# olivesgatech/R3D

Hardware: AMD Instinct MI355X
Metric: training clips/sec (RGB+Depth fusion, DARai) at 1/2/4/8 GPUs; effective-rank match (higher is better)
Workload: dtype f32 (depth products: bf16x3 split on the bf16 matrix cores, fp32 accumulate)

## Files before the change

r3d_amd/csrc/decoder_chain.hip:

```cpp
#include "chain_bf3.h"
#include "mha_small.h"
#include "losses_dev.h"

namespace r3d {

constexpr int kDcBufA = 0;
constexpr int kDcBufB = kDcBufA + kFcRows * kFcP1;
constexpr int kDcBufF = kDcBufB + kFcRows * kFcP1;
constexpr int kDcWl = kDcBufF + kFcRows * kFcP4;
constexpr int kDcWlWave = 128 * kFbWP;
constexpr int kDcRed = kDcWl + 8 * kDcWlWave;
constexpr int kDcLdsFloats = kDcRed + 2 * 2 * 8 * kFcRows;
constexpr int kDcLdsBytes = kDcLdsFloats * 4;
static_assert(16 * kFcWP <= kDcWlWave && mha_small_lds_floats(16, 8) <= kDcWlWave && mha_small_bwd_lds_floats(16, 8) <= kDcWlWave,
              "wave region");
static_assert(kDcLdsBytes + (2 * 8 * (kTLHeads + 8) + 8 * 4 * 128 + 64) * 4 <= 160 * 1024, "LDS (dynamic + the tail's static arrays)");

typedef r3d_decoder_chain_args DcArgs;

__device__ __forceinline__ void dc_stage_rows(float* buf, const float* src, int row0, int tid) {
    const int r = tid >> 5, c4 = tid & 31;
    const f32x4 z = {0.f, 0.f, 0.f, 0.f};
    const f32x4 v = *reinterpret_cast<const f32x4*>(src + (size_t)(row0 + (r & 7)) * kFcH + 4 * c4);
    *reinterpret_cast<f32x4*>(buf + r * kFcP1 + 4 * c4) = r < 8 ? v : z;
// ... 427 lines not shown
            if (CHIP) relu |= (f > 0.f ? 1u : 0u) << (4 * t + i);
        }
    }
    if (CHIP) {
        keep.relu = relu;
#pragma unroll
        for (int t = 0; t < 4; ++t)
            keep.kbf[t] = kbf[t];
    }
    __syncthreads();
    R3D_CHAIN_MARK(D.timeline, b == 0, 5);
    acc0 = zero; acc1 = zero;
    bf3_chunk<4>(imgF, kD3P4, li, q, 0, b2, acc0, acc1);
    __builtin_amdgcn_sched_barrier(0);
    bf3_bload<4>(b2, D.pl_w2, 16, wave, 12, lane);
    __builtin_amdgcn_sched_barrier(0);
    bf3_chunk<4>(imgF, kD3P4, li, q, 4, b0, acc0, acc1);
    bf3_chunk<4>(imgF, kD3P4, li, q, 8, b1, acc0, acc1);
    bf3_chunk<4>(imgF, kD3P4, li, q, 12, b2, acc0, acc1);
    if (live) {
#pragma unroll
        for (int i = 0; i < 4; ++i) {
            const float v = ((acc0[i] + acc1[i]) + b_2) * md3.keep((uint8_t)(kb3 >> (8 * i)), D.drop_scale) + t2v[i];
            D.t3_pre[(size_t)(row0 + 4 * q + i) * H + c] = v;
            if (CHIP) scr0[kD3Xt + (4 * q + i) * H + c] = v;
        }
    }
}

struct Dc3TailIo {
    static constexpr bool kChip = true;
    float* scr0; unsigned short* imgA; const unsigned short* pl_w2_t; int tid_, wave, lane;
    Bf3B& w0; Bf3B& w1;
    __device__ __forceinline__ int tid() const { return tid_; }
    __device__ __forceinline__ float x(int row, int c) const { return scr0[kD3Xt + row * kFcH + c]; }
    __device__ __forceinline__ float ln(int which, int c) const { return scr0[kD3Par + which * kFcH + c]; }
    __device__ __forceinline__ float wh(int k, int c) const { return scr0[kD3ParWh + k * kFcH + c]; }
    __device__ __forceinline__ float bh(int k) const { return scr0[kD3ParBh + k]; }
    __device__ __forceinline__ void grads(int row, int c, float dx, float dx2) const {
        scr0[kD3Dxt + row * kFcH + c] = dx;
        asm volatile("" : "+v"(dx2));
        bf3_store1(imgA, kD3P1, row, c, dx2);
    }
    __device__ __forceinline__ void loads_requested() const {
        bf3_bload<4>(w0, pl_w2_t, 4, 4 * wave + 0, 0, lane);
        bf3_bload<4>(w1, pl_w2_t, 4, 4 * wave + 1, 0, lane);
    }
};

template <bool CHIP>
__device__ __forceinline__ void dc3_bwd(const DcArgs& D, const int b_, float* lds, const Dc3Keep& keep, Bf3B& b0, Bf3B& b1, Bf3B& b2) {
    int tid = threadIdx.x, b = b_;
    if (CHIP) { asm volatile("" : "+v"(tid)); asm volatile("" : "+s"(b)); }
    const int lane = tid & 63, wave = tid >> 6;
    const int li = lane & 15, q = lane >> 4;
    unsigned short* img = reinterpret_cast<unsigned short*>(lds);
    unsigned short* imgA = img + kD3ImgA;
    unsigned short* imgF = img + kD3ImgF;
    float* dct = reinterpret_cast<float*>(img + kD3ImgB);
    float* scr0 = reinterpret_cast<float*>(reinterpret_cast<unsigned char*>(lds) + kD3ScrBytes);
    float* scr = scr0 + wave * kD3ScrWave;
    float* redA = reinterpret_cast<float*>(reinterpret_cast<unsigned char*>(lds) + kD3RedBytes);
    constexpr int H = kFcH;
    const int row0 = b * 8;
    const int c = wave * 16 + li;
    const bool live = q < 2;
    const f32x4 zero = {0.f, 0.f, 0.f, 0.f};
// ... 102 lines not shown
            const float o = r2v[i] * (g[i] - s1v[i] - xh[i] * s2v[i]);
            const size_t e = (size_t)(row0 + 4 * q + i) * H + c;
            const float ok = o * md2.keep(kb2[i], D.drop_scale);
            if (live) { D.d_t2pre[e] = o; D.d_cap[e] = ok; }
            bf3_store1(imgA, kD3P1, 4 * q + i, c, live ? ok : 0.f);
        }
    }
    __syncthreads();
    R3D_CHAIN_MARK(D.timeline, b == 0, 13);
    acc0 = zero; acc1 = zero;
    bf3_chunk<4>(imgA, kD3P1, li, q, 0, b2, acc0, acc1);
    if (live) {
#pragma unroll
        for (int i = 0; i < 4; ++i) {
            const float v = acc0[i] + acc1[i];
            D.d_cao[(size_t)(row0 + 4 * q + i) * H + c] = v;
            if (CHIP) dct[(4 * q + i) * H + c] = v;
        }
    }
    R3D_CHAIN_MARK(D.timeline, b == 0, 14);
    __syncthreads();
    if (CHIP) {
        mha_bwd_small_compute<16, 8, false, true>(m, b * 8 + wave, scr, mr, dct, H, lane);
    } else {
        mha_bwd_small_unit<16, 8, false>(m, b * 8 + wave, scr);
    }
    R3D_CHAIN_MARK(D.timeline, b == 0, 15);
}

__global__ __launch_bounds__(512) void decoder_chain_bf3_kernel(const DcArgs D, const r3d_tail_losses_args t, const LossArgs a,
                                                                float* part, unsigned* arrivals) {
    extern __shared__ __attribute__((aligned(16))) float lds[];
    __shared__ float lg[8][kTLHeads + 8];
    __shared__ float dl[8][kTLHeads + 8];
    __shared__ float red[8][4][128];
    __shared__ int is_last;
    if (threadIdx.x >= 256) __builtin_amdgcn_s_setprio(0); else __builtin_amdgcn_s_setprio(2);
    const int lane = threadIdx.x & 63, wave = threadIdx.x >> 6;
    if ((int)blockIdx.x < D.B) {
        const int b = (int)blockIdx.x;
        Dc3Keep keep{};
        Bf3B w0, w1, w2;
        if (D.phases == 7) {
            dc3_fwd<true>(D, t, b, lds, keep);
            R3D_CHAIN_MARK(D.timeline, b == 0, 6);
            __syncthreads();
            float* scr0 = reinterpret_cast<float*>(reinterpret_cast<unsigned char*>(lds) + kD3ScrBytes);
            int tid2 = threadIdx.x;
            asm volatile("" : "+v"(tid2));
            tail_clip_body(t, a, part, b, lg, dl, red,
                           Dc3TailIo{scr0, reinterpret_cast<unsigned short*>(lds) + kD3ImgA, D.pl_w2_t, tid2, tid2 >> 6, tid2 & 63,
                                     w0, w1});
            R3D_CHAIN_MARK(D.timeline, b == 0, 7);
            dc3_bwd<true>(D, b, lds, keep, w0, w1, w2);
        } else {
            if (D.phases & 1) dc3_fwd<false>(D, t, b, lds, keep);
            R3D_CHAIN_MARK(D.timeline, b == 0, 6);
            if (D.phases & 2) {
                __syncthreads();
                tail_clip_body(t, a, part, b, lg, dl, red);
            }
            R3D_CHAIN_MARK(D.timeline, b == 0, 7);
            if (D.phases & 4) {
                __syncthreads();
                dc3_bwd<false>(D, b, lds, keep, w0, w1, w2);
            }
        }
    } else if (D.phases & 2) {
        const int u = ((int)blockIdx.x - D.B) * 8 + wave;
        if (u < a.B * a.S) losses_unit(a, part, u, lane);
    }
    if (D.phases & 2) tail_losses_finish(t, a, part, arrivals, &is_last);
}

__global__ __launch_bounds__(512) void decoder_chain_kernel(const DcArgs D, const r3d_tail_losses_args t, const LossArgs a,
                                                            float* part, unsigned* arrivals) {
    extern __shared__ __attribute__((aligned(16))) float lds[];
    if (threadIdx.x >= 256) __builtin_amdgcn_s_setprio(0); else __builtin_amdgcn_s_setprio(2);
    __shared__ float lg[8][kTLHeads + 8];
    __shared__ float dl[8][kTLHeads + 8];
    __shared__ float red[8][4][128];
    __shared__ int is_last;
    const int lane = threadIdx.x & 63, wave = threadIdx.x >> 6;
    if ((int)blockIdx.x < D.B) {
        const int b = (int)blockIdx.x;
        if (D.phases & 1) dc_fwd(D, b, lds);
        R3D_CHAIN_MARK(D.timeline, b == 0, 6);
        if (D.phases & 2) {
            __syncthreads();
            tail_clip_body(t, a, part, b, lg, dl, red);
        }
        R3D_CHAIN_MARK(D.timeline, b == 0, 7);
        if (D.phases & 4) {
            __syncthreads();
            dc_bwd(D, b, lds);
        }
    } else if (D.phases & 2) {
        const int u = ((int)blockIdx.x - D.B) * 8 + wave;
        if (u < a.B * a.S) losses_unit(a, part, u, lane);
    }
    if (D.phases & 2) tail_losses_finish(t, a, part, arrivals, &is_last);
}

}

using namespace r3d;

R3D_EXPORT int r3d_decoder_tail_losses_supported(int H, int n_head, int Q, int rows);

R3D_EXPORT int r3d_decoder_chain_supported(int H, int Q, int heads, int S) {
    return (H == kFcH && Q == 8 && heads == 8 && S > 0 && S <= 64) ? 1 : 0;
}

R3D_EXPORT int r3d_decoder_chain(const r3d_decoder_chain_args* d, const r3d_tail_losses_args* tail, float* ws, void* stream) {
    R3D_REQUIRE(d && (d->phases & 7) && !(d->phases & ~7));
    R3D_REQUIRE(r3d_decoder_chain_supported(d->H, d->Q, d->heads, d->S) && d->B > 0);
    R3D_REQUIRE(d->caq && d->cakv && d->p_ca && d->wo && d->w1 && d->w2 && d->t2_pre && d->m2 && d->r2 && d->g2 && d->ff1);
    if (d->phases & 1)
        R3D_REQUIRE(d->ca_o && d->bo && d->t1 && d->be2 && d->t2 && d->b1 && d->b2 && d->t3_pre);
    if (d->phases & 4)
        R3D_REQUIRE(d->d_t3pre && d->d_ff2 && d->d_ff1 && d->d_t2pre && d->d_cap && d->d_cao && d->d_caq && d->d_cakv && d->part_d2);
    const void* al[] = {d->caq, d->cakv, d->wo, d->w1, d->w2, d->ca_o, d->d_ff2, d->d_cao, d->d_cakv};
    for (const void* p : al)
// ... 41 lines not shown
```

r3d_amd/csrc/losses.hip:

```cpp
#include "losses_dev.h"
#include "loss_finalize.h"

namespace r3d {

__global__ __launch_bounds__(256) void losses_kernel(const LossArgs a, float* part, unsigned* arrivals) {
    __shared__ int is_last;
    const int lane = threadIdx.x & 63;
    const int u = blockIdx.x * 4 + (threadIdx.x >> 6);
    if (u < a.B * a.S + a.B * a.Q + a.B) losses_unit(a, part, u, lane);
    __builtin_amdgcn_s_waitcnt(0);
    __syncthreads();
    if (threadIdx.x == 0)
        is_last = (__hip_atomic_fetch_add(arrivals, 1u, __ATOMIC_RELAXED, __HIP_MEMORY_SCOPE_AGENT) == gridDim.x - 1) ? 1 : 0;
    __syncthreads();
    if (!is_last) return;
    losses_finalize(a, part);
    if (threadIdx.x == 0) *arrivals = 0u;
}


__global__ __launch_bounds__(512) void tail_losses_kernel(const r3d_tail_losses_args t, const LossArgs a, float* part,
                                                          unsigned* arrivals) {
    __shared__ float lg[8][kTLHeads + 8];
    __shared__ float dl[8][kTLHeads + 8];
    __shared__ float red[8][4][128];
    __shared__ int is_last;
    const int lane = threadIdx.x & 63, wave = threadIdx.x >> 6;
    if ((int)blockIdx.x < a.B) {
        tail_clip_body(t, a, part, (int)blockIdx.x, lg, dl, red);
    } else {
        const int u = ((int)blockIdx.x - a.B) * 8 + wave;
        if (u < a.B * a.S) losses_unit(a, part, u, lane);
    }
    tail_losses_finish(t, a, part, arrivals, &is_last);
}

__global__ __launch_bounds__(512) void tail_losses_wide_kernel(const r3d_tail_losses_args t, const LossArgs a, float* part,
                                                               unsigned* arrivals) {
    extern __shared__ __attribute__((aligned(16))) float dyn[];
    __shared__ float lg[8][kTLHeads + 8];
    __shared__ float dl[8][kTLHeads + 8];
    __shared__ int is_last;
    const int lane = threadIdx.x & 63, wave = threadIdx.x >> 6;
    if ((int)blockIdx.x < a.B) {
        float* whs = dyn;
        float* red = dyn + (size_t)t.n_head * t.H;
        for (int i = threadIdx.x; i < t.n_head * t.H; i += 512) whs[i] = t.w_head[i];
        __syncthreads();
        tail_clip_body_wide<8>(t, a, part, (int)blockIdx.x, lg, dl, whs, red);
    } else {
        const int u = ((int)blockIdx.x - a.B) * 8 + wave;
        if (u < a.B * a.S) losses_unit(a, part, u, lane);
    }
    tail_losses_finish(t, a, part, arrivals, &is_last);
}

__global__ __launch_bounds__(256) void losses_finalize_kernel(const r3d_loss_finalize_job j) {
    __shared__ double red[4][3][3];
    loss_finalize_block<4>(j, red);
}

}
// ... 159 lines not shown
```

r3d_amd/csrc/losses_dev.h:

```cpp
#pragma once
#include "common.h"
#include "../../include/r3d_hip.h"

namespace r3d {

struct LossArgs {
    const float* seg; int ld_seg; const float* act; int ld_act; const float* dur; int ld_dur;
    const int64_t* past_label; const int64_t* target; const float* target_dur;
    int B, S, Q, K, pad_idx, exclude_idx; int val_mode;
    const float* dur_den; float grad_scale;
    float* d_seg; int ld_dseg; float* d_act; int ld_dact; float* d_dur; int ld_ddur;
    float* loss_out; int64_t* counts;
    int64_t* tick_a; int64_t* tick_b;
    int Kseg = 0;
};

__device__ __forceinline__ float ce_row(const float* logit, int K, int64_t label, bool valid, int pad_idx,
                                        float gscale, float* dl, int lane, int* argmax_out) {
    float m = -INFINITY;
    int am = 0x7fffffff;
    if (K <= 64) {
        const float x = lane < K ? logit[lane] : -INFINITY;
        m = wave_max(x);
        const unsigned long long hit = __ballot(lane < K && x == m);
// ... 179 lines not shown
            if (lane == 0) red8[wave][g][k] = t;
        }
    __syncthreads();
    if (threadIdx.x == 0) {
        double t[3][3];
        for (int g = 0; g < 3; ++g)
            for (int k = 0; k < 3; ++k)
                t[g][k] = ((red8[0][g][k] + red8[1][g][k]) + (red8[2][g][k] + red8[3][g][k])) +
                          ((red8[4][g][k] + red8[5][g][k]) + (red8[6][g][k] + red8[7][g][k]));
        const double msum = t[2][2] / (double)a.B;
        const double dur_den = a.dur_den ? (double)*a.dur_den : msum;
        const float ls = a.seg ? (float)(t[0][0] / (double)N) : 0.f;
        const float la = (float)(t[1][0] / (double)BQ);
        const float ld = (float)(t[2][0] / dur_den);
        a.loss_out[0] = ls; a.loss_out[1] = la; a.loss_out[2] = ld; a.loss_out[3] = ls + la + ld;
        a.counts[0] = (int64_t)(t[0][1] + 0.5); a.counts[1] = (int64_t)(t[0][2] + 0.5);
        a.counts[2] = (int64_t)(t[1][1] + 0.5); a.counts[3] = (int64_t)(t[1][2] + 0.5);
        if (a.tick_a) *a.tick_a += 1;
        if (a.tick_b) *a.tick_b += 1;
    }
}

constexpr int kTLHeads = 24;

struct TailGlobalIo {
    static constexpr bool kChip = false;
    __device__ __forceinline__ int tid() const { return threadIdx.x; }
    __device__ __forceinline__ float x(int, int) const { return 0.f; }
    __device__ __forceinline__ float ln(int, int) const { return 0.f; }
    __device__ __forceinline__ float wh(int, int) const { return 0.f; }
    __device__ __forceinline__ float bh(int) const { return 0.f; }
    __device__ __forceinline__ void grads(int, int, float, float) const {}
    __device__ __forceinline__ void loads_requested() const {}
};

template <class Io = TailGlobalIo>
__device__ __forceinline__ void tail_clip_body(const r3d_tail_losses_args& t, const LossArgs& a, float* part, const int b,
                                               float (*lg)[kTLHeads + 8], float (*dl)[kTLHeads + 8], float (*red)[4][128],
                                               const Io io = Io()) {
    const int tid = io.tid(), lane = tid & 63, wave = tid >> 6;
    const int H = t.H, K = a.K, Q = a.Q, NH = t.n_head, N = a.B * a.S, BQ = a.B * a.Q;
    const int row = b * Q + wave;
    int cc[2];
    float x[2], g3[2], b3[2], gF[2], bF[2];
#pragma unroll
    for (int e = 0; e < 2; ++e) {
        const int c = lane + 64 * e;
        cc[e] = c < H ? c : H - 1;
        if (Io::kChip) {
            x[e] = io.x(wave, cc[e]);
            g3[e] = io.ln(0, cc[e]); b3[e] = io.ln(1, cc[e]); gF[e] = io.ln(2, cc[e]); bF[e] = io.ln(3, cc[e]);
        } else {
            x[e] = t.x[(size_t)row * H + cc[e]];
            g3[e] = t.g3[cc[e]]; b3[e] = t.b3[cc[e]]; gF[e] = t.gF[cc[e]]; bF[e] = t.bF[cc[e]];
        }
    }
    float wh[kTLHeads][2];
#pragma unroll
    for (int k = 0; k < kTLHeads; ++k) {
        const int kc = k < NH ? k : NH - 1;
#pragma unroll
        for (int e = 0; e < 2; ++e) wh[k][e] = Io::kChip ? io.wh(kc, cc[e]) : t.w_head[(size_t)kc * H + cc[e]];
    }
    float keep[2];
    uint8_t keep_raw[2] = {0, 0};
    if (Io::kChip) {
        const uint8_t* dp = t.drop ? t.drop + (size_t)row * H : reinterpret_cast<const uint8_t*>(t.g3);
#pragma unroll
        for (int e = 0; e < 2; ++e) keep_raw[e] = dp[cc[e]];
    } else {
#pragma unroll
        for (int e = 0; e < 2; ++e) keep[e] = t.drop ? t.drop_scale * (float)t.drop[(size_t)row * H + cc[e]] : 1.f;
    }
    const bool small = a.S <= 64 && BQ <= 64;
    const int64_t pl_pre = a.past_label[(size_t)b * a.S + (lane < a.S ? lane : 0)];
    const int64_t tgt_first = a.target[(size_t)b * Q];
    const int64_t tgt_row = a.target[row];
    const float td_all = a.target_dur[lane < BQ ? lane : 0];
    const float td_clip = a.target_dur[(size_t)b * Q + (lane < Q ? lane : 0)];
    const float* ddp = a.dur_den ? a.dur_den : t.g3;
    const float dden_pre = Io::kChip ? *ddp : (a.dur_den ? *a.dur_den : 0.f);
    io.loads_requested();
    if (Io::kChip) {
#pragma unroll
        for (int e = 0; e < 2; ++e) keep[e] = t.drop ? t.drop_scale * (float)keep_raw[e] : 1.f;
    }
    float y3[2], yF[2], m3, r3, mF, rF;
    ln2_apply(x, g3, b3, H, lane, y3, m3, r3);
    ln2_apply(y3, gF, bF, H, lane, yF, mF, rF);
    if (lane == 0) { t.m3[row] = m3; t.r3[row] = r3; t.mF[row] = mF; t.rF[row] = rF; }
#pragma unroll
    for (int e = 0; e < 2; ++e)
        if (lane + 64 * e < H) {
            t.t3[(size_t)row * H + lane + 64 * e] = y3[e];
            t.tgtF[(size_t)row * H + lane + 64 * e] = yF[e];
        }
    {
        float p[kTLHeads];
#pragma unroll
        for (int k = 0; k < kTLHeads; ++k) p[k] = yF[0] * wh[k][0] + yF[1] * wh[k][1];
#pragma unroll
        for (int k = 0; k < kTLHeads; ++k) {
            if (k < NH) {
                const float v = wave_sum(p[k]) + (Io::kChip ? io.bh(k) : t.b_head[k]);
                if (lane == 0) { t.out[(size_t)row * t.ld_out + k] = v; lg[wave][k] = v; }
            }
        }
    }
    __syncthreads();
    float out_l, out_c, out_v;
    {
        int last = -1;
        int64_t ref = (int64_t)a.pad_idx;
        if (small) {
            const unsigned long long obs = __ballot(lane < a.S && pl_pre != (int64_t)a.pad_idx);
            last = obs ? 63 - __builtin_clzll(obs) : -1;
            const int lsel = __builtin_amdgcn_readfirstlane(last < 0 ? 0 : last);
            const unsigned rlo = __builtin_amdgcn_readlane((unsigned)(unsigned long long)pl_pre, lsel);
            const unsigned rhi = __builtin_amdgcn_readlane((unsigned)((unsigned long long)pl_pre >> 32), lsel);
            if (last >= 0) ref = (int64_t)(((unsigned long long)rhi << 32) | rlo);
        } else {
            for (int s = lane; s < a.S; s += 64)
                if (a.past_label[(size_t)b * a.S + s] != (int64_t)a.pad_idx) last = s;
#pragma unroll
            for (int off = 32; off > 0; off >>= 1) last = max(last, __shfl_xor(last, off, 64));
            if (last >= 0) ref = a.past_label[(size_t)b * a.S + last];
        }
        const float w = (ref == tgt_first) ? 1.0f : 10.0f;
        const int64_t lab = tgt_row;
        const bool valid = (lab != (int64_t)a.pad_idx) && (lab != (int64_t)a.exclude_idx) && lab >= 0 && lab < K;
        int am;
        const float l = ce_row(&lg[wave][0], K, lab, valid, a.pad_idx, w * a.grad_scale / (float)BQ, &dl[wave][0], lane, &am);
        out_l = l * w; out_v = valid ? 1.f : 0.f; out_c = (valid && (int64_t)am == lab) ? 1.f : 0.f;
        if (lane == 0) {
            __hip_atomic_store(part + 4 * (size_t)(N + row) + 0, out_l, __ATOMIC_RELAXED, __HIP_MEMORY_SCOPE_AGENT);
            __hip_atomic_store(part + 4 * (size_t)(N + row) + 1, out_c, __ATOMIC_RELAXED, __HIP_MEMORY_SCOPE_AGENT);
            __hip_atomic_store(part + 4 * (size_t)(N + row) + 2, out_v, __ATOMIC_RELAXED, __HIP_MEMORY_SCOPE_AGENT);
// ... 7 lines not shown
        mc = wave_sum(mc);
        const float dur_den = a.dur_den ? dden_pre : mc;
        const float mkq = (lane < Q && td_clip != (float)a.pad_idx) ? 1.f : 0.f;
        const float eq = lane < Q ? expf(lg[lane < Q ? lane : 0][K]) * mkq : 0.f;
        const float ssum = wave_sum(fabsf(eq));
        const float den = fmaxf(ssum, 1e-12f);
        float sq = 0.f, gp = 0.f;
        if (lane < Q) {
            const float p = eq / den;
            const float tt = td_clip * mkq * mkq;
            const float diff = p - tt;
            sq = diff * diff;
            gp = (2.f * diff / dur_den) * p;
        }
        sq = wave_sum(sq);
        gp = wave_sum(gp);
        const float td_w = __builtin_bit_cast(float, __builtin_amdgcn_readlane(__builtin_bit_cast(unsigned, td_clip),
                                                                               __builtin_amdgcn_readfirstlane(wave)));
        if (lane == 0) {
            const float td = td_w;
            const float mk = (td != (float)a.pad_idx) ? 1.f : 0.f;
            const float p = expf(lg[wave][K]) * mk / den;
            const float g = 2.f * (p - td * mk * mk) / dur_den;
            dl[wave][K] = ((ssum >= 1e-12f) ? p * (g - gp) : 0.f) * a.grad_scale;
            if (wave == 0) {
                const size_t u = (size_t)N + BQ + b;
                __hip_atomic_store(part + 4 * u + 0, sq, __ATOMIC_RELAXED, __HIP_MEMORY_SCOPE_AGENT);
                __hip_atomic_store(part + 4 * u + 1, 0.f, __ATOMIC_RELAXED, __HIP_MEMORY_SCOPE_AGENT);
                __hip_atomic_store(part + 4 * u + 2, mc, __ATOMIC_RELAXED, __HIP_MEMORY_SCOPE_AGENT);
            }
        }
    }
    for (int k = lane; k < NH; k += 64) t.d_out[(size_t)row * t.ld_dout + k] = dl[wave][k];
    float d[2] = {0.f, 0.f};
#pragma unroll
    for (int k = 0; k < kTLHeads; ++k) {
        if (k < NH) {
            const float dk = dl[wave][k];
            d[0] += dk * wh[k][0]; d[1] += dk * wh[k][1];
        }
    }
    float agF[2], abF[2], ag3[2], ab3[2], xh[2], gg[2], s1 = 0.f, s2 = 0.f;
#pragma unroll
    for (int e = 0; e < 2; ++e) {
        const bool in = lane + 64 * e < H;
        xh[e] = in ? (y3[e] - mF) * rF : 0.f;
        const float dd = in ? d[e] : 0.f;
        agF[e] = dd * xh[e]; abF[e] = dd;
        gg[e] = dd * gF[e];
        s1 += gg[e]; s2 += gg[e] * xh[e];
    }
    s1 = wave_sum(s1) / (float)H; s2 = wave_sum(s2) / (float)H;
    float dt[2], u1 = 0.f, u2 = 0.f;
#pragma unroll
    for (int e = 0; e < 2; ++e) dt[e] = rF * (gg[e] - s1 - xh[e] * s2);
#pragma unroll
    for (int e = 0; e < 2; ++e) {
        const bool in = lane + 64 * e < H;
        xh[e] = in ? (x[e] - m3) * r3 : 0.f;
        const float dd = in ? dt[e] : 0.f;
        ag3[e] = dd * xh[e]; ab3[e] = dd;
        gg[e] = dd * g3[e];
        u1 += gg[e]; u2 += gg[e] * xh[e];
    }
    u1 = wave_sum(u1) / (float)H; u2 = wave_sum(u2) / (float)H;
#pragma unroll
    for (int e = 0; e < 2; ++e) {
        const int c = lane + 64 * e;
        if (c < H) {
            const float o = r3 * (gg[e] - u1 - xh[e] * u2);
            t.dx[(size_t)row * H + c] = o;
            t.dx2[(size_t)row * H + c] = o * keep[e];
            io.grads(wave, c, o, o * keep[e]);
            red[wave][0][c] = agF[e]; red[wave][1][c] = abF[e]; red[wave][2][c] = ag3[e]; red[wave][3][c] = ab3[e];
        }
    }
    __syncthreads();
    for (int i = threadIdx.x; i < 2 * 4 * H; i += 512) {
        const int half = i / (4 * H), j = i - half * 4 * H, which = j / H, c = j - which * H;
        const int w0 = 4 * half;
        const float s = (red[w0][which][c] + red[w0 + 1][which][c]) + (red[w0 + 2][which][c] + red[w0 + 3][which][c]);
        float* ws = which < 2 ? t.wsF : t.ws3;
        ws[((size_t)(2 * b + half) * 2 + (which & 1)) * H + c] = s;
    }
}

template <int EPL>
__device__ __forceinline__ void lnw_apply(const float (&x)[EPL], const float (&g)[EPL], const float (&b)[EPL], int H, int lane,
                                          float (&y)[EPL], float& mean, float& rstd) {
    float s = 0.f;
#pragma unroll
    for (int e = 0; e < EPL; ++e) s += (lane + 64 * e < H) ? x[e] : 0.f;
    mean = wave_sum(s) / (float)H;
    float q = 0.f;
#pragma unroll
    for (int e = 0; e < EPL; ++e) {
        const float dl = (lane + 64 * e < H) ? x[e] - mean : 0.f;
        q += dl * dl;
    }
    rstd = 1.0f / sqrtf(wave_sum(q) / (float)H + kLnEpsTL);
#pragma unroll
    for (int e = 0; e < EPL; ++e) y[e] = (lane + 64 * e < H) ? (x[e] - mean) * rstd * g[e] + b[e] : 0.f;
}

template <int EPL>
__device__ __forceinline__ void tail_clip_body_wide(const r3d_tail_losses_args& t, const LossArgs& a, float* part, const int b,
                                                    float (*lg)[kTLHeads + 8], float (*dl)[kTLHeads + 8], const float* whs,
                                                    float* red) {
    const int lane = threadIdx.x & 63, wave = threadIdx.x >> 6;
    const int H = t.H, K = a.K, Q = a.Q, NH = t.n_head, N = a.B * a.S, BQ = a.B * a.Q;
    const int row = b * Q + wave;
    int cc[EPL];
    float x[EPL], g3[EPL], b3[EPL], gF[EPL], bF[EPL];
#pragma unroll
    for (int e = 0; e < EPL; ++e) {
        const int c = lane + 64 * e;
        cc[e] = c < H ? c : H - 1;
        x[e] = t.x[(size_t)row * H + cc[e]];
        g3[e] = t.g3[cc[e]]; b3[e] = t.b3[cc[e]]; gF[e] = t.gF[cc[e]]; bF[e] = t.bF[cc[e]];
    }
    float keep[EPL];
#pragma unroll
    for (int e = 0; e < EPL; ++e) keep[e] = t.drop ? t.drop_scale * (float)t.drop[(size_t)row * H + cc[e]] : 1.f;
    const bool small = a.S <= 64 && BQ <= 64;
    const int64_t pl_pre = a.past_label[(size_t)b * a.S + (lane < a.S ? lane : 0)];
    const int64_t tgt_first = a.target[(size_t)b * Q];
    const int64_t tgt_row = a.target[row];
    const float td_all = a.target_dur[lane < BQ ? lane : 0];
    const float td_clip = a.target_dur[(size_t)b * Q + (lane < Q ? lane : 0)];
    const float dden_pre = a.dur_den ? *a.dur_den : 0.f;
    float y3[EPL], yF[EPL], m3, r3, mF, rF;
    lnw_apply<EPL>(x, g3, b3, H, lane, y3, m3, r3);
    lnw_apply<EPL>(y3, gF, bF, H, lane, yF, mF, rF);
    if (lane == 0) { t.m3[row] = m3; t.r3[row] = r3; t.mF[row] = mF; t.rF[row] = rF; }
#pragma unroll
    for (int e = 0; e < EPL; ++e)
        if (lane + 64 * e < H) {
            t.t3[(size_t)row * H + lane + 64 * e] = y3[e];
            t.tgtF[(size_t)row * H + lane + 64 * e] = yF[e];
        }
    {
        float p[kTLHeads];
#pragma unroll
        for (int k = 0; k < kTLHeads; ++k) {
            const int kc = k < NH ? k : NH - 1;
            float s = 0.f;
#pragma unroll
            for (int e = 0; e < EPL; ++e) s += yF[e] * whs[(size_t)kc * H + cc[e]];
            p[k] = s;
        }
#pragma unroll
        for (int k = 0; k < kTLHeads; ++k) {
            if (k < NH) {
                const float v = wave_sum(p[k]) + t.b_head[k];
                if (lane == 0) { t.out[(size_t)row * t.ld_out + k] = v; lg[wave][k] = v; }
            }
        }
    }
    __syncthreads();
    float out_l, out_c, out_v;
    {
        int last = -1;
        int64_t ref = (int64_t)a.pad_idx;
        if (small) {
            const unsigned long long obs = __ballot(lane < a.S && pl_pre != (int64_t)a.pad_idx);
            last = obs ? 63 - __builtin_clzll(obs) : -1;
            const int lsel = __builtin_amdgcn_readfirstlane(last < 0 ? 0 : last);
            const unsigned rlo = __builtin_amdgcn_readlane((unsigned)(unsigned long long)pl_pre, lsel);
            const unsigned rhi = __builtin_amdgcn_readlane((unsigned)((unsigned long long)pl_pre >> 32), lsel);
            if (last >= 0) ref = (int64_t)(((unsigned long long)rhi << 32) | rlo);
        } else {
            for (int s = lane; s < a.S; s += 64)
                if (a.past_label[(size_t)b * a.S + s] != (int64_t)a.pad_idx) last = s;
#pragma unroll
            for (int off = 32; off > 0; off >>= 1) last = max(last, __shfl_xor(last, off, 64));
            if (last >= 0) ref = a.past_label[(size_t)b * a.S + last];
        }
        const float w = (ref == tgt_first) ? 1.0f : 10.0f;
        const int64_t lab = tgt_row;
        const bool valid = (lab != (int64_t)a.pad_idx) && (lab != (int64_t)a.exclude_idx) && lab >= 0 && lab < K;
        int am;
        const float l = ce_row(&lg[wave][0], K, lab, valid, a.pad_idx, w * a.grad_scale / (float)BQ, &dl[wave][0], lane, &am);
        out_l = l * w; out_v = valid ? 1.f : 0.f; out_c = (valid && (int64_t)am == lab) ? 1.f : 0.f;
        if (lane == 0) {
            __hip_atomic_store(part + 4 * (size_t)(N + row) + 0, out_l, __ATOMIC_RELAXED, __HIP_MEMORY_SCOPE_AGENT);
            __hip_atomic_store(part + 4 * (size_t)(N + row) + 1, out_c, __ATOMIC_RELAXED, __HIP_MEMORY_SCOPE_AGENT);
            __hip_atomic_store(part + 4 * (size_t)(N + row) + 2, out_v, __ATOMIC_RELAXED, __HIP_MEMORY_SCOPE_AGENT);
        }
    }
    {
        float mc = 0.f;
        if (small) mc = (lane < BQ && td_all != (float)a.pad_idx) ? 1.f : 0.f;
        else
            for (int e = lane; e < BQ; e += 64) mc += (a.target_dur[e] != (float)a.pad_idx) ? 1.f : 0.f;
        mc = wave_sum(mc);
        const float dur_den = a.dur_den ? dden_pre : mc;
        const float mkq = (lane < Q && td_clip != (float)a.pad_idx) ? 1.f : 0.f;
        const float eq = lane < Q ? expf(lg[lane < Q ? lane : 0][K]) * mkq : 0.f;
        const float ssum = wave_sum(fabsf(eq));
        const float den = fmaxf(ssum, 1e-12f);
        float sq = 0.f, gp = 0.f;
        if (lane < Q) {
            const float p = eq / den;
            const float tt = td_clip * mkq * mkq;
            const float diff = p - tt;
            sq = diff * diff;
            gp = (2.f * diff / dur_den) * p;
        }
        sq = wave_sum(sq);
        gp = wave_sum(gp);
        const float td_w = __builtin_bit_cast(float, __builtin_amdgcn_readlane(__builtin_bit_cast(unsigned, td_clip),
                                                                               __builtin_amdgcn_readfirstlane(wave)));
        if (lane == 0) {
            const float td = td_w;
            const float mk = (td != (float)a.pad_idx) ? 1.f : 0.f;
            const float p = expf(lg[wave][K]) * mk / den;
            const float g = 2.f * (p - td * mk * mk) / dur_den;
            dl[wave][K] = ((ssum >= 1e-12f) ? p * (g - gp) : 0.f) * a.grad_scale;
            if (wave == 0) {
                const size_t u = (size_t)N + BQ + b;
                __hip_atomic_store(part + 4 * u + 0, sq, __ATOMIC_RELAXED, __HIP_MEMORY_SCOPE_AGENT);
                __hip_atomic_store(part + 4 * u + 1, 0.f, __ATOMIC_RELAXED, __HIP_MEMORY_SCOPE_AGENT);
                __hip_atomic_store(part + 4 * u + 2, mc, __ATOMIC_RELAXED, __HIP_MEMORY_SCOPE_AGENT);
            }
        }
    }
    for (int k = lane; k < NH; k += 64) t.d_out[(size_t)row * t.ld_dout + k] = dl[wave][k];
    float d[EPL];
#pragma unroll
    for (int e = 0; e < EPL; ++e) d[e] = 0.f;
#pragma unroll
    for (int k = 0; k < kTLHeads; ++k) {
        if (k < NH) {
            const float dk = dl[wave][k];
#pragma unroll
            for (int e = 0; e < EPL; ++e) d[e] += dk * whs[(size_t)k * H + cc[e]];
        }
    }
    float agF[EPL], abF[EPL], ag3[EPL], ab3[EPL], xh[EPL], gg[EPL], s1 = 0.f, s2 = 0.f;
#pragma unroll
    for (int e = 0; e < EPL; ++e) {
        const bool in = lane + 64 * e < H;
        xh[e] = in ? (y3[e] - mF) * rF : 0.f;
        const float dd = in ? d[e] : 0.f;
        agF[e] = dd * xh[e]; abF[e] = dd;
        gg[e] = dd * gF[e];
        s1 += gg[e]; s2 += gg[e] * xh[e];
    }
    s1 = wave_sum(s1) / (float)H; s2 = wave_sum(s2) / (float)H;
    float dt[EPL], u1 = 0.f, u2 = 0.f;
#pragma unroll
    for (int e = 0; e < EPL; ++e) dt[e] = rF * (gg[e] - s1 - xh[e] * s2);
#pragma unroll
    for (int e = 0; e < EPL; ++e) {
        const bool in = lane + 64 * e < H;
        xh[e] = in ? (x[e] - m3) * r3 : 0.f;
        const float dd = in ? dt[e] : 0.f;
        ag3[e] = dd * xh[e]; ab3[e] = dd;
        gg[e] = dd * g3[e];
        u1 += gg[e]; u2 += gg[e] * xh[e];
// ... 45 lines not shown
```

Measured before the change: 46080.

## Register-resident tail head: scatter-reduce logits, CE and dur grads without LDS dl

```diff
diff --git a/r3d_amd/csrc/decoder_chain.hip b/r3d_amd/csrc/decoder_chain.hip
--- a/r3d_amd/csrc/decoder_chain.hip
+++ b/r3d_amd/csrc/decoder_chain.hip
@@ -483,7 +483,9 @@
     static constexpr bool kChip = true;
     float* scr0; unsigned short* imgA; const unsigned short* pl_w2_t; int tid_, wave, lane;
     Bf3B& w0; Bf3B& w1;
+    uint64_t* timeline; bool marks;
     __device__ __forceinline__ int tid() const { return tid_; }
+    __device__ __forceinline__ void mark(int k) const { R3D_CHAIN_MARK(timeline, marks, k); }
     __device__ __forceinline__ float x(int row, int c) const { return scr0[kD3Xt + row * kFcH + c]; }
     __device__ __forceinline__ float ln(int which, int c) const { return scr0[kD3Par + which * kFcH + c]; }
     __device__ __forceinline__ float wh(int k, int c) const { return scr0[kD3ParWh + k * kFcH + c]; }
@@ -652,7 +654,6 @@
                                                                 float* part, unsigned* arrivals) {
     extern __shared__ __attribute__((aligned(16))) float lds[];
     __shared__ float lg[8][kTLHeads + 8];
-    __shared__ float dl[8][kTLHeads + 8];
     __shared__ float red[8][4][128];
     __shared__ int is_last;
     if (threadIdx.x >= 256) __builtin_amdgcn_s_setprio(0); else __builtin_amdgcn_s_setprio(2);
@@ -668,9 +669,9 @@
             float* scr0 = reinterpret_cast<float*>(reinterpret_cast<unsigned char*>(lds) + kD3ScrBytes);
             int tid2 = threadIdx.x;
             asm volatile("" : "+v"(tid2));
-            tail_clip_body(t, a, part, b, lg, dl, red,
+            tail_clip_body(t, a, part, b, lg, red,
                            Dc3TailIo{scr0, reinterpret_cast<unsigned short*>(lds) + kD3ImgA, D.pl_w2_t, tid2, tid2 >> 6, tid2 & 63,
-                                     w0, w1});
+                                     w0, w1, D.timeline, b == 0});
             R3D_CHAIN_MARK(D.timeline, b == 0, 7);
             dc3_bwd<true>(D, b, lds, keep, w0, w1, w2);
         } else {
@@ -678,7 +679,7 @@
             R3D_CHAIN_MARK(D.timeline, b == 0, 6);
             if (D.phases & 2) {
                 __syncthreads();
-                tail_clip_body(t, a, part, b, lg, dl, red);
+                tail_clip_body(t, a, part, b, lg, red);
             }
             R3D_CHAIN_MARK(D.timeline, b == 0, 7);
             if (D.phases & 4) {
@@ -698,7 +699,6 @@
     extern __shared__ __attribute__((aligned(16))) float lds[];
     if (threadIdx.x >= 256) __builtin_amdgcn_s_setprio(0); else __builtin_amdgcn_s_setprio(2);
     __shared__ float lg[8][kTLHeads + 8];
-    __shared__ float dl[8][kTLHeads + 8];
     __shared__ float red[8][4][128];
     __shared__ int is_last;
     const int lane = threadIdx.x & 63, wave = threadIdx.x >> 6;
@@ -708,7 +708,7 @@
         R3D_CHAIN_MARK(D.timeline, b == 0, 6);
         if (D.phases & 2) {
             __syncthreads();
-            tail_clip_body(t, a, part, b, lg, dl, red);
+            tail_clip_body(t, a, part, b, lg, red);
         }
         R3D_CHAIN_MARK(D.timeline, b == 0, 7);
         if (D.phases & 4) {
diff --git a/r3d_amd/csrc/losses.hip b/r3d_amd/csrc/losses.hip
--- a/r3d_amd/csrc/losses.hip
+++ b/r3d_amd/csrc/losses.hip
@@ -22,12 +22,11 @@
 __global__ __launch_bounds__(512) void tail_losses_kernel(const r3d_tail_losses_args t, const LossArgs a, float* part,
                                                           unsigned* arrivals) {
     __shared__ float lg[8][kTLHeads + 8];
-    __shared__ float dl[8][kTLHeads + 8];
     __shared__ float red[8][4][128];
     __shared__ int is_last;
     const int lane = threadIdx.x & 63, wave = threadIdx.x >> 6;
     if ((int)blockIdx.x < a.B) {
-        tail_clip_body(t, a, part, (int)blockIdx.x, lg, dl, red);
+        tail_clip_body(t, a, part, (int)blockIdx.x, lg, red);
     } else {
         const int u = ((int)blockIdx.x - a.B) * 8 + wave;
         if (u < a.B * a.S) losses_unit(a, part, u, lane);
diff --git a/r3d_amd/csrc/losses_dev.h b/r3d_amd/csrc/losses_dev.h
--- a/r3d_amd/csrc/losses_dev.h
+++ b/r3d_amd/csrc/losses_dev.h
@@ -235,12 +235,38 @@
     __device__ __forceinline__ float bh(int) const { return 0.f; }
     __device__ __forceinline__ void grads(int, int, float, float) const {}
     __device__ __forceinline__ void loads_requested() const {}
+    __device__ __forceinline__ void mark(int) const {}
 };
+
+__device__ __forceinline__ float dpp_xor4_f(float v) {
+    const int s = __builtin_bit_cast(int, v);
+    int r = __builtin_amdgcn_update_dpp(0, s, 0x104, 0xf, 0x5, false);
+    r = __builtin_amdgcn_update_dpp(r, s, 0x114, 0xf, 0xa, false);
+    return __builtin_bit_cast(float, r);
+}
+__device__ __forceinline__ float wave_sum32_scatter(const float (&p)[32], int lane) {
+    float v16[16], v8[8], v4[4], v2[2];
+    const bool h8 = lane & 8, h4 = lane & 4, h2 = lane & 2, h1 = lane & 1;
+#pragma unroll
+    for (int k = 0; k < 16; ++k) v16[k] = (h8 ? p[k + 16] : p[k]) + dpp_mov_f<0x128>(h8 ? p[k] : p[k + 16]);
+#pragma unroll
+    for (int k = 0; k < 8; ++k) v8[k] = (h4 ? v16[k + 8] : v16[k]) + dpp_xor4_f(h4 ? v16[k] : v16[k + 8]);
+#pragma unroll
+    for (int k = 0; k < 4; ++k) v4[k] = (h2 ? v8[k + 4] : v8[k]) + dpp_mov_f<0x4E>(h2 ? v8[k] : v8[k + 4]);
+#pragma unroll
+    for (int k = 0; k < 2; ++k) v2[k] = (h1 ? v4[k + 2] : v4[k]) + dpp_mov_f<0xB1>(h1 ? v4[k] : v4[k + 2]);
+    const auto r = __builtin_amdgcn_permlane16_swap(__builtin_bit_cast(unsigned, v2[0]), __builtin_bit_cast(unsigned, v2[1]),
+                                                    false, false);
+    const unsigned r0 = r[0], r1 = r[1];
+    const float w = __builtin_bit_cast(float, r0) + __builtin_bit_cast(float, r1);
+    const auto q = __builtin_amdgcn_permlane32_swap(__builtin_bit_cast(unsigned, w), __builtin_bit_cast(unsigned, w), false, false);
+    const unsigned q0 = q[0], q1 = q[1];
+    return __builtin_bit_cast(float, q0) + __builtin_bit_cast(float, q1);
+}
 
 template <class Io = TailGlobalIo>
 __device__ __forceinline__ void tail_clip_body(const r3d_tail_losses_args& t, const LossArgs& a, float* part, const int b,
-                                               float (*lg)[kTLHeads + 8], float (*dl)[kTLHeads + 8], float (*red)[4][128],
-                                               const Io io = Io()) {
+                                               float (*lg)[kTLHeads + 8], float (*red)[4][128], const Io io = Io()) {
     const int tid = io.tid(), lane = tid & 63, wave = tid >> 6;
     const int H = t.H, K = a.K, Q = a.Q, NH = t.n_head, N = a.B * a.S, BQ = a.B * a.Q;
     const int row = b * Q + wave;
@@ -265,6 +291,9 @@
 #pragma unroll
         for (int e = 0; e < 2; ++e) wh[k][e] = Io::kChip ? io.wh(kc, cc[e]) : t.w_head[(size_t)kc * H + cc[e]];
     }
+    const int hl = ((lane & 15) << 1) | ((lane >> 4) & 1);
+    const int hlc = hl < NH ? hl : NH - 1;
+    const float bh_l = Io::kChip ? io.bh(hlc) : t.b_head[hlc];
     float keep[2];
     uint8_t keep_raw[2] = {0, 0};
     if (Io::kChip) {
@@ -299,13 +328,219 @@
             t.tgtF[(size_t)row * H + lane + 64 * e] = yF[e];
         }
     {
+        float p[32];
+#pragma unroll
+        for (int k = 0; k < kTLHeads; ++k) p[k] = __builtin_fmaf(yF[0], wh[k][0], yF[1] * wh[k][1]);
+#pragma unroll
+        for (int k = kTLHeads; k < 32; ++k) p[k] = 0.f;
+        const float v = wave_sum32_scatter(p, lane) + bh_l;
+        if (lane < 32 && hl < NH) { t.out[(size_t)row * t.ld_out + hl] = v; lg[wave][hl] = v; }
+    }
+    __syncthreads();
+    io.mark(8);
+    const float xv = lg[wave][lane < NH ? lane : 0];
+    const float dq = lg[lane < Q ? lane : 0][K];
+    float out_l, out_c, out_v, gce;
+    {
+        int last = -1;
+        int64_t ref = (int64_t)a.pad_idx;
+        if (small) {
+            const unsigned long long obs = __ballot(lane < a.S && pl_pre != (int64_t)a.pad_idx);
+            last = obs ? 63 - __builtin_clzll(obs) : -1;
+            const int lsel = __builtin_amdgcn_readfirstlane(last < 0 ? 0 : last);
+            const unsigned rlo = __builtin_amdgcn_readlane((unsigned)(unsigned long long)pl_pre, lsel);
+            const unsigned rhi = __builtin_amdgcn_readlane((unsigned)((unsigned long long)pl_pre >> 32), lsel);
+            if (last >= 0) ref = (int64_t)(((unsigned long long)rhi << 32) | rlo);
+        } else {
+            for (int s = lane; s < a.S; s += 64)
+                if (a.past_label[(size_t)b * a.S + s] != (int64_t)a.pad_idx) last = s;
+#pragma unroll
+            for (int off = 32; off > 0; off >>= 1) last = max(last, __shfl_xor(last, off, 64));
+            if (last >= 0) ref = a.past_label[(size_t)b * a.S + last];
+        }
+        const float w = (ref == tgt_first) ? 1.0f : 10.0f;
+        const int64_t lab = tgt_row;
+        const bool valid = (lab != (int64_t)a.pad_idx) && (lab != (int64_t)a.exclude_idx) && lab >= 0 && lab < K;
+        const float gscale = w * a.grad_scale / (float)BQ;
+        const bool cls = lane < K;
+        const float xc = cls ? xv : -INFINITY;
+        const float m = wave_max(xc);
+        const unsigned long long hit = __ballot(cls && xc == m);
+        const int am = hit ? __builtin_ctzll(hit) : 0x7fffffff;
+        const float se = wave_sum(cls ? expf(xv - m) : 0.f);
+        const float lse = m + logf(se);
+        const float xl = readlane_f(xv, __builtin_amdgcn_readfirstlane(valid ? (int)lab : 0));
+        const float l = valid ? lse - xl : 0.f;
+        gce = (valid && cls) ? (expf(xv - lse) - ((int64_t)lane == lab ? 1.f : 0.f)) * gscale : 0.f;
+        out_l = l * w; out_v = valid ? 1.f : 0.f; out_c = (valid && (int64_t)am == lab) ? 1.f : 0.f;
+    }
+    float g_l;
+    {
+        float mc = 0.f;
+        if (small) mc = (lane < BQ && td_all != (float)a.pad_idx) ? 1.f : 0.f;
+        else
+            for (int e = lane; e < BQ; e += 64) mc += (a.target_dur[e] != (float)a.pad_idx) ? 1.f : 0.f;
+        mc = wave_sum(mc);
+        const float dur_den = a.dur_den ? dden_pre : mc;
+        const float mkq = (lane < Q && td_clip != (float)a.pad_idx) ? 1.f : 0.f;
+        const float eq = lane < Q ? expf(dq) * mkq : 0.f;
+        const float ssum = wave_sum(fabsf(eq));
+        const float den = fmaxf(ssum, 1e-12f);
+        const float p = eq / den;
+        const float diff = lane < Q ? p - td_clip * mkq * mkq : 0.f;
+        const float gq = lane < Q ? 2.f * diff / dur_den : 0.f;
+        float sq = diff * diff, gp = gq * p;
+        asm volatile("" : "+v"(sq));
+        asm volatile("" : "+v"(gp));
+        sq = wave_sum(sq);
+        gp = wave_sum(gp);
+        const float dd = ((ssum >= 1e-12f) ? p * (gq - gp) : 0.f) * a.grad_scale;
+        const float dd_w = readlane_f(dd, __builtin_amdgcn_readfirstlane(wave));
+        g_l = lane < K ? gce : (lane == K ? dd_w : 0.f);
+        if (lane == 0) {
+            __hip_atomic_store(part + 4 * (size_t)(N + row) + 0, out_l, __ATOMIC_RELAXED, __HIP_MEMORY_SCOPE_AGENT);
+            __hip_atomic_store(part + 4 * (size_t)(N + row) + 1, out_c, __ATOMIC_RELAXED, __HIP_MEMORY_SCOPE_AGENT);
+            __hip_atomic_store(part + 4 * (size_t)(N + row) + 2, out_v, __ATOMIC_RELAXED, __HIP_MEMORY_SCOPE_AGENT);
+            if (wave == 0) {
+                const size_t u = (size_t)N + BQ + b;
+                __hip_atomic_store(part + 4 * u + 0, sq, __ATOMIC_RELAXED, __HIP_MEMORY_SCOPE_AGENT);
+                __hip_atomic_store(part + 4 * u + 1, 0.f, __ATOMIC_RELAXED, __HIP_MEMORY_SCOPE_AGENT);
+                __hip_atomic_store(part + 4 * u + 2, mc, __ATOMIC_RELAXED, __HIP_MEMORY_SCOPE_AGENT);
+            }
+        }
+    }
+    if (lane < NH) t.d_out[(size_t)row * t.ld_dout + lane] = g_l;
+    float d[2] = {0.f, 0.f};
+#pragma unroll
+    for (int k = 0; k < kTLHeads; ++k) {
+        const float dk = readlane_f(g_l, k);
+        d[0] = __builtin_fmaf(dk, wh[k][0], d[0]); d[1] = __builtin_fmaf(dk, wh[k][1], d[1]);
+    }
+    float agF[2], abF[2], ag3[2], ab3[2], xh[2], gg[2], s1 = 0.f, s2 = 0.f;
+#pragma unroll
+    for (int e = 0; e < 2; ++e) {
+        const bool in = lane + 64 * e < H;
+        xh[e] = in ? (y3[e] - mF) * rF : 0.f;
+        const float dd = in ? d[e] : 0.f;
+        agF[e] = dd * xh[e]; abF[e] = dd;
+        gg[e] = dd * gF[e];
+        s1 += gg[e]; s2 += gg[e] * xh[e];
+    }
+    s1 = wave_sum(s1) / (float)H; s2 = wave_sum(s2) / (float)H;
+    float dt[2], u1 = 0.f, u2 = 0.f;
+#pragma unroll
+    for (int e = 0; e < 2; ++e) dt[e] = rF * (gg[e] - s1 - xh[e] * s2);
+#pragma unroll
+    for (int e = 0; e < 2; ++e) {
+        const bool in = lane + 64 * e < H;
+        xh[e] = in ? (x[e] - m3) * r3 : 0.f;
+        const float dd = in ? dt[e] : 0.f;
+        ag3[e] = dd * xh[e]; ab3[e] = dd;
+        gg[e] = dd * g3[e];
+        u1 += gg[e]; u2 += gg[e] * xh[e];
+    }
+    u1 = wave_sum(u1) / (float)H; u2 = wave_sum(u2) / (float)H;
+#pragma unroll
+    for (int e = 0; e < 2; ++e) {
+        const int c = lane + 64 * e;
+        if (c < H) {
+            const float o = r3 * (gg[e] - u1 - xh[e] * u2);
+            t.dx[(size_t)row * H + c] = o;
+            t.dx2[(size_t)row * H + c] = o * keep[e];
+            io.grads(wave, c, o, o * keep[e]);
+            red[wave][0][c] = agF[e]; red[wave][1][c] = abF[e]; red[wave][2][c] = ag3[e]; red[wave][3][c] = ab3[e];
+        }
+    }
+    io.mark(9);
+    __syncthreads();
+    if (H == 128) {
+        const int which = tid >> 7, c = tid & 127;
+        float* ws = which < 2 ? t.wsF : t.ws3;
+#pragma unroll
+        for (int half = 0; half < 2; ++half) {
+            const int w0 = 4 * half;
+            const float s = (red[w0][which][c] + red[w0 + 1][which][c]) + (red[w0 + 2][which][c] + red[w0 + 3][which][c]);
+            ws[((size_t)(2 * b + half) * 2 + (which & 1)) * 128 + c] = s;
+        }
+    } else {
+        for (int i = tid; i < 2 * 4 * H; i += 512) {
+            const int half = i / (4 * H), j = i - half * 4 * H, which = j / H, c = j - which * H;
+            const int w0 = 4 * half;
+            const float s = (red[w0][which][c] + red[w0 + 1][which][c]) + (red[w0 + 2][which][c] + red[w0 + 3][which][c]);
+            float* ws = which < 2 ? t.wsF : t.ws3;
+            ws[((size_t)(2 * b + half) * 2 + (which & 1)) * H + c] = s;
+        }
+    }
+}
+
+template <int EPL>
+__device__ __forceinline__ void lnw_apply(const float (&x)[EPL], const float (&g)[EPL], const float (&b)[EPL], int H, int lane,
+                                          float (&y)[EPL], float& mean, float& rstd) {
+    float s = 0.f;
+#pragma unroll
+    for (int e = 0; e < EPL; ++e) s += (lane + 64 * e < H) ? x[e] : 0.f;
+    mean = wave_sum(s) / (float)H;
+    float q = 0.f;
+#pragma unroll
+    for (int e = 0; e < EPL; ++e) {
+        const float dl = (lane + 64 * e < H) ? x[e] - mean : 0.f;
+        q += dl * dl;
+    }
+    rstd = 1.0f / sqrtf(wave_sum(q) / (float)H + kLnEpsTL);
+#pragma unroll
+    for (int e = 0; e < EPL; ++e) y[e] = (lane + 64 * e < H) ? (x[e] - mean) * rstd * g[e] + b[e] : 0.f;
+}
+
+template <int EPL>
+__device__ __forceinline__ void tail_clip_body_wide(const r3d_tail_losses_args& t, const LossArgs& a, float* part, const int b,
+                                                    float (*lg)[kTLHeads + 8], float (*dl)[kTLHeads + 8], const float* whs,
+                                                    float* red) {
+    const int lane = threadIdx.x & 63, wave = threadIdx.x >> 6;
+    const int H = t.H, K = a.K, Q = a.Q, NH = t.n_head, N = a.B * a.S, BQ = a.B * a.Q;
+    const int row = b * Q + wave;
+    int cc[EPL];
+    float x[EPL], g3[EPL], b3[EPL], gF[EPL], bF[EPL];
+#pragma unroll
+    for (int e = 0; e < EPL; ++e) {
+        const int c = lane + 64 * e;
+        cc[e] = c < H ? c : H - 1;
+        x[e] = t.x[(size_t)row * H + cc[e]];
+        g3[e] = t.g3[cc[e]]; b3[e] = t.b3[cc[e]]; gF[e] = t.gF[cc[e]]; bF[e] = t.bF[cc[e]];
+    }
+    float keep[EPL];
+#pragma unroll
+    for (int e = 0; e < EPL; ++e) keep[e] = t.drop ? t.drop_scale * (float)t.drop[(size_t)row * H + cc[e]] : 1.f;
+    const bool small = a.S <= 64 && BQ <= 64;
+    const int64_t pl_pre = a.past_label[(size_t)b * a.S + (lane < a.S ? lane : 0)];
+    const int64_t tgt_first = a.target[(size_t)b * Q];
+    const int64_t tgt_row = a.target[row];
+    const float td_all = a.target_dur[lane < BQ ? lane : 0];
+    const float td_clip = a.target_dur[(size_t)b * Q + (lane < Q ? lane : 0)];
+    const float dden_pre = a.dur_den ? *a.dur_den : 0.f;
+    float y3[EPL], yF[EPL], m3, r3, mF, rF;
+    lnw_apply<EPL>(x, g3, b3, H, lane, y3, m3, r3);
+    lnw_apply<EPL>(y3, gF, bF, H, lane, yF, mF, rF);
+    if (lane == 0) { t.m3[row] = m3; t.r3[row] = r3; t.mF[row] = mF; t.rF[row] = rF; }
+#pragma unroll
+    for (int e = 0; e < EPL; ++e)
+        if (lane + 64 * e < H) {
+            t.t3[(size_t)row * H + lane + 64 * e] = y3[e];
+            t.tgtF[(size_t)row * H + lane + 64 * e] = yF[e];
+        }
+    {
         float p[kTLHeads];
 #pragma unroll
-        for (int k = 0; k < kTLHeads; ++k) p[k] = yF[0] * wh[k][0] + yF[1] * wh[k][1];
+        for (int k = 0; k < kTLHeads; ++k) {
+            const int kc = k < NH ? k : NH - 1;
+            float s = 0.f;
+#pragma unroll
+            for (int e = 0; e < EPL; ++e) s += yF[e] * whs[(size_t)kc * H + cc[e]];
+            p[k] = s;
+        }
 #pragma unroll
         for (int k = 0; k < kTLHeads; ++k) {
             if (k < NH) {
-                const float v = wave_sum(p[k]) + (Io::kChip ? io.bh(k) : t.b_head[k]);
+                const float v = wave_sum(p[k]) + t.b_head[k];
                 if (lane == 0) { t.out[(size_t)row * t.ld_out + k] = v; lg[wave][k] = v; }
             }
         }
@@ -379,200 +614,6 @@
         }
     }
     for (int k = lane; k < NH; k += 64) t.d_out[(size_t)row * t.ld_dout + k] = dl[wave][k];
-    float d[2] = {0.f, 0.f};
-#pragma unroll
-    for (int k = 0; k < kTLHeads; ++k) {
-        if (k < NH) {
-            const float dk = dl[wave][k];
-            d[0] += dk * wh[k][0]; d[1] += dk * wh[k][1];
-        }
-    }
-    float agF[2], abF[2], ag3[2], ab3[2], xh[2], gg[2], s1 = 0.f, s2 = 0.f;
-#pragma unroll
-    for (int e = 0; e < 2; ++e) {
-        const bool in = lane + 64 * e < H;
-        xh[e] = in ? (y3[e] - mF) * rF : 0.f;
-        const float dd = in ? d[e] : 0.f;
-        agF[e] = dd * xh[e]; abF[e] = dd;
-        gg[e] = dd * gF[e];
-        s1 += gg[e]; s2 += gg[e] * xh[e];
-    }
-    s1 = wave_sum(s1) / (float)H; s2 = wave_sum(s2) / (float)H;
-    float dt[2], u1 = 0.f, u2 = 0.f;
-#pragma unroll
-    for (int e = 0; e < 2; ++e) dt[e] = rF * (gg[e] - s1 - xh[e] * s2);
-#pragma unroll
-    for (int e = 0; e < 2; ++e) {
-        const bool in = lane + 64 * e < H;
-        xh[e] = in ? (x[e] - m3) * r3 : 0.f;
-        const float dd = in ? dt[e] : 0.f;
-        ag3[e] = dd * xh[e]; ab3[e] = dd;
-        gg[e] = dd * g3[e];
-        u1 += gg[e]; u2 += gg[e] * xh[e];
-    }
-    u1 = wave_sum(u1) / (float)H; u2 = wave_sum(u2) / (float)H;
-#pragma unroll
-    for (int e = 0; e < 2; ++e) {
-        const int c = lane + 64 * e;
-        if (c < H) {
-            const float o = r3 * (gg[e] - u1 - xh[e] * u2);
-            t.dx[(size_t)row * H + c] = o;
-            t.dx2[(size_t)row * H + c] = o * keep[e];
-            io.grads(wave, c, o, o * keep[e]);
-            red[wave][0][c] = agF[e]; red[wave][1][c] = abF[e]; red[wave][2][c] = ag3[e]; red[wave][3][c] = ab3[e];
-        }
-    }
-    __syncthreads();
-    for (int i = threadIdx.x; i < 2 * 4 * H; i += 512) {
-        const int half = i / (4 * H), j = i - half * 4 * H, which = j / H, c = j - which * H;
-        const int w0 = 4 * half;
-        const float s = (red[w0][which][c] + red[w0 + 1][which][c]) + (red[w0 + 2][which][c] + red[w0 + 3][which][c]);
-        float* ws = which < 2 ? t.wsF : t.ws3;
-        ws[((size_t)(2 * b + half) * 2 + (which & 1)) * H + c] = s;
-    }
-}
-
-template <int EPL>
-__device__ __forceinline__ void lnw_apply(const float (&x)[EPL], const float (&g)[EPL], const float (&b)[EPL], int H, int lane,
-                                          float (&y)[EPL], float& mean, float& rstd) {
-    float s = 0.f;
-#pragma unroll
-    for (int e = 0; e < EPL; ++e) s += (lane + 64 * e < H) ? x[e] : 0.f;
-    mean = wave_sum(s) / (float)H;
-    float q = 0.f;
-#pragma unroll
-    for (int e = 0; e < EPL; ++e) {
-        const float dl = (lane + 64 * e < H) ? x[e] - mean : 0.f;
-        q += dl * dl;
-    }
-    rstd = 1.0f / sqrtf(wave_sum(q) / (float)H + kLnEpsTL);
-#pragma unroll
-    for (int e = 0; e < EPL; ++e) y[e] = (lane + 64 * e < H) ? (x[e] - mean) * rstd * g[e] + b[e] : 0.f;
-}
-
-template <int EPL>
-__device__ __forceinline__ void tail_clip_body_wide(const r3d_tail_losses_args& t, const LossArgs& a, float* part, const int b,
-                                                    float (*lg)[kTLHeads + 8], float (*dl)[kTLHeads + 8], const float* whs,
-                                                    float* red) {
-    const int lane = threadIdx.x & 63, wave = threadIdx.x >> 6;
-    const int H = t.H, K = a.K, Q = a.Q, NH = t.n_head, N = a.B * a.S, BQ = a.B * a.Q;
-    const int row = b * Q + wave;
-    int cc[EPL];
-    float x[EPL], g3[EPL], b3[EPL], gF[EPL], bF[EPL];
-#pragma unroll
-    for (int e = 0; e < EPL; ++e) {
-        const int c = lane + 64 * e;
-        cc[e] = c < H ? c : H - 1;
-        x[e] = t.x[(size_t)row * H + cc[e]];
-        g3[e] = t.g3[cc[e]]; b3[e] = t.b3[cc[e]]; gF[e] = t.gF[cc[e]]; bF[e] = t.bF[cc[e]];
-    }
-    float keep[EPL];
-#pragma unroll
-    for (int e = 0; e < EPL; ++e) keep[e] = t.drop ? t.drop_scale * (float)t.drop[(size_t)row * H + cc[e]] : 1.f;
-    const bool small = a.S <= 64 && BQ <= 64;
-    const int64_t pl_pre = a.past_label[(size_t)b * a.S + (lane < a.S ? lane : 0)];
-    const int64_t tgt_first = a.target[(size_t)b * Q];
-    const int64_t tgt_row = a.target[row];
-    const float td_all = a.target_dur[lane < BQ ? lane : 0];
-    const float td_clip = a.target_dur[(size_t)b * Q + (lane < Q ? lane : 0)];
-    const float dden_pre = a.dur_den ? *a.dur_den : 0.f;
-    float y3[EPL], yF[EPL], m3, r3, mF, rF;
-    lnw_apply<EPL>(x, g3, b3, H, lane, y3, m3, r3);
-    lnw_apply<EPL>(y3, gF, bF, H, lane, yF, mF, rF);
-    if (lane == 0) { t.m3[row] = m3; t.r3[row] = r3; t.mF[row] = mF; t.rF[row] = rF; }
-#pragma unroll
-    for (int e = 0; e < EPL; ++e)
-        if (lane + 64 * e < H) {
-            t.t3[(size_t)row * H + lane + 64 * e] = y3[e];
-            t.tgtF[(size_t)row * H + lane + 64 * e] = yF[e];
-        }
-    {
-        float p[kTLHeads];
-#pragma unroll
-        for (int k = 0; k < kTLHeads; ++k) {
-            const int kc = k < NH ? k : NH - 1;
-            float s = 0.f;
-#pragma unroll
-            for (int e = 0; e < EPL; ++e) s += yF[e] * whs[(size_t)kc * H + cc[e]];
-            p[k] = s;
-        }
-#pragma unroll
-        for (int k = 0; k < kTLHeads; ++k) {
-            if (k < NH) {
-                const float v = wave_sum(p[k]) + t.b_head[k];
-                if (lane == 0) { t.out[(size_t)row * t.ld_out + k] = v; lg[wave][k] = v; }
-            }
-        }
-    }
-    __syncthreads();
-    float out_l, out_c, out_v;
-    {
-        int last = -1;
-        int64_t ref = (int64_t)a.pad_idx;
-        if (small) {
-            const unsigned long long obs = __ballot(lane < a.S && pl_pre != (int64_t)a.pad_idx);
-            last = obs ? 63 - __builtin_clzll(obs) : -1;
-            const int lsel = __builtin_amdgcn_readfirstlane(last < 0 ? 0 : last);
-            const unsigned rlo = __builtin_amdgcn_readlane((unsigned)(unsigned long long)pl_pre, lsel);
-            const unsigned rhi = __builtin_amdgcn_readlane((unsigned)((unsigned long long)pl_pre >> 32), lsel);
-            if (last >= 0) ref = (int64_t)(((unsigned long long)rhi << 32) | rlo);
-        } else {
-            for (int s = lane; s < a.S; s += 64)
-                if (a.past_label[(size_t)b * a.S + s] != (int64_t)a.pad_idx) last = s;
-#pragma unroll
-            for (int off = 32; off > 0; off >>= 1) last = max(last, __shfl_xor(last, off, 64));
-            if (last >= 0) ref = a.past_label[(size_t)b * a.S + last];
-        }
-        const float w = (ref == tgt_first) ? 1.0f : 10.0f;
-        const int64_t lab = tgt_row;
-        const bool valid = (lab != (int64_t)a.pad_idx) && (lab != (int64_t)a.exclude_idx) && lab >= 0 && lab < K;
-        int am;
-        const float l = ce_row(&lg[wave][0], K, lab, valid, a.pad_idx, w * a.grad_scale / (float)BQ, &dl[wave][0], lane, &am);
-        out_l = l * w; out_v = valid ? 1.f : 0.f; out_c = (valid && (int64_t)am == lab) ? 1.f : 0.f;
-        if (lane == 0) {
-            __hip_atomic_store(part + 4 * (size_t)(N + row) + 0, out_l, __ATOMIC_RELAXED, __HIP_MEMORY_SCOPE_AGENT);
-            __hip_atomic_store(part + 4 * (size_t)(N + row) + 1, out_c, __ATOMIC_RELAXED, __HIP_MEMORY_SCOPE_AGENT);
-            __hip_atomic_store(part + 4 * (size_t)(N + row) + 2, out_v, __ATOMIC_RELAXED, __HIP_MEMORY_SCOPE_AGENT);
-        }
-    }
-    {
-        float mc = 0.f;
-        if (small) mc = (lane < BQ && td_all != (float)a.pad_idx) ? 1.f : 0.f;
-        else
-            for (int e = lane; e < BQ; e += 64) mc += (a.target_dur[e] != (float)a.pad_idx) ? 1.f : 0.f;
-        mc = wave_sum(mc);
-        const float dur_den = a.dur_den ? dden_pre : mc;
-        const float mkq = (lane < Q && td_clip != (float)a.pad_idx) ? 1.f : 0.f;
-        const float eq = lane < Q ? expf(lg[lane < Q ? lane : 0][K]) * mkq : 0.f;
-        const float ssum = wave_sum(fabsf(eq));
-        const float den = fmaxf(ssum, 1e-12f);
-        float sq = 0.f, gp = 0.f;
-        if (lane < Q) {
-            const float p = eq / den;
-            const float tt = td_clip * mkq * mkq;
-            const float diff = p - tt;
-            sq = diff * diff;
-            gp = (2.f * diff / dur_den) * p;
-        }
-        sq = wave_sum(sq);
-        gp = wave_sum(gp);
-        const float td_w = __builtin_bit_cast(float, __builtin_amdgcn_readlane(__builtin_bit_cast(unsigned, td_clip),
-                                                                               __builtin_amdgcn_readfirstlane(wave)));
-        if (lane == 0) {
-            const float td = td_w;
-            const float mk = (td != (float)a.pad_idx) ? 1.f : 0.f;
-            const float p = expf(lg[wave][K]) * mk / den;
-            const float g = 2.f * (p - td * mk * mk) / dur_den;
-            dl[wave][K] = ((ssum >= 1e-12f) ? p * (g - gp) : 0.f) * a.grad_scale;
-            if (wave == 0) {
-                const size_t u = (size_t)N + BQ + b;
-                __hip_atomic_store(part + 4 * u + 0, sq, __ATOMIC_RELAXED, __HIP_MEMORY_SCOPE_AGENT);
-                __hip_atomic_store(part + 4 * u + 1, 0.f, __ATOMIC_RELAXED, __HIP_MEMORY_SCOPE_AGENT);
-                __hip_atomic_store(part + 4 * u + 2, mc, __ATOMIC_RELAXED, __HIP_MEMORY_SCOPE_AGENT);
-            }
-        }
-    }
-    for (int k = lane; k < NH; k += 64) t.d_out[(size_t)row * t.ld_dout + k] = dl[wave][k];
     float d[EPL];
 #pragma unroll
     for (int e = 0; e < EPL; ++e) d[e] = 0.f;
```

New measurement: 46880, median of 6. +1.7%, better.
